# bensonlzl/spaced-kmer-sketching

Measured on AMD Instinct MI355X. Metric: k-mers hashed/s + genome-pairs ANI/s at 1/2/4/8 MI355X; % HBM roofline, higher is better.
Workload: dtype u64; 1 GPU; config3: 1x3 Gb multi-contig genome per GPU, spaced seed w=31/k=21 (mask seed 0), FracMinHash 1/1000; builds_in_flight=3, genome_bytes=3000000024, windows_per_genome=2999036400, sketch_size=2998764, parallelism=genome-sharded x1

## Files before the change

### spaced-kmer-sketching_amd/csrc/scan.hip

```cpp
#include <hip/hip_runtime.h>

#include <cstdlib>

#include <cstdint>
#include <type_traits>

#include "sks_hash.hpp"
#include "sks_internal.hpp"

namespace sks {

namespace {

constexpr int kBlock = 256;
constexpr int kWPT = 16;
constexpr int kTile = kBlock * kWPT;
constexpr int kHaloWords = 4;
constexpr int kWords = kBlock + kHaloWords;
constexpr int kLoadVecs = (kWords * 16 + 16) / 16;
constexpr int kQCap = 2048;
#ifndef SKS_SCAN_QCAP
#define SKS_SCAN_QCAP 512
#endif
template <int MODE>
constexpr int qcap() { return MODE == kModeList ? kQCap : SKS_SCAN_QCAP; }
constexpr unsigned char kSep = '\n';

struct Geom {
  uint64_t win0;
  uint64_t seg_end;
  uint32_t seg;
};

__device__ __forceinline__ Geom tile_geom(const ScanParams& p, uint64_t tile, uint32_t& seg) {
  while (seg + 1 < p.n_seg && tile >= p.tile_prefix[seg + 1]) ++seg;
  Geom g;
  g.seg = seg;
  g.win0 = p.seg_begin[seg] + (tile - p.tile_prefix[seg]) * (uint64_t)kTile;
  g.seg_end = p.seg_end[seg];
  return g;
}

__device__ __forceinline__ uint4 load_vec(const uint8_t* __restrict__ seq, int64_t base, int k,
                                          int64_t seg_end) {
  int64_t a = base + 16 * (int64_t)k;
  if (a + 16 <= seg_end) return *reinterpret_cast<const uint4*>(seq + a);
  uint32_t wv[4];
#pragma unroll
  for (int q = 0; q < 4; ++q) {
    uint32_t v = 0;
#pragma unroll
    for (int b = 0; b < 4; ++b) {
      int64_t pos = a + 4 * q + b;
      uint32_t ch = pos < seg_end ? seq[pos] : kSep;
      v |= ch << (8 * b);
    }
    wv[q] = v;
  }
  return make_uint4(wv[0], wv[1], wv[2], wv[3]);
}

__device__ __forceinline__ uint32_t align_shift(const uint8_t* seq, uint64_t win0) {
  return (uint32_t)(((uintptr_t)seq + win0) & 15u);
}

__device__ __forceinline__ void encode4(uint32_t x, uint32_t& le8, uint32_t& inv4) {
  uint32_t low = x | 0x20202020u;
  uint32_t code = ((low >> 1) ^ (low >> 2)) & 0x03030303u;
  uint32_t expect = __builtin_amdgcn_perm(0u, 0x74676361u, code);
  uint32_t eq = expect ^ low;
  uint32_t t = (eq & 0x7F7F7F7Fu) + 0x7F7F7F7Fu;
  t = ~(t | eq | 0x7F7F7F7Fu);
  uint32_t bad = (~t) & 0x80808080u;
  inv4 = (bad * 0x00204081u) >> 28;
  uint32_t y = code | (code >> 6);
  le8 = (y | (y >> 12)) & 0xFFu;
}

__device__ __forceinline__ uint32_t funnel(uint32_t hi, uint32_t lo, uint32_t s) {
  return __builtin_amdgcn_alignbit(hi, lo, s);
}

template <bool ALIGNED>
__device__ __forceinline__ void pack16(const uint32_t (&x)[5], uint32_t sb, uint32_t& le,
                                       uint32_t& inv) {
  uint32_t w[4], g[4], sad = 0;
#pragma unroll
  for (int k = 0; k < 4; ++k) {
    w[k] = ALIGNED ? x[k] : funnel(x[k + 1], x[k], sb);
    const uint32_t low = w[k] | 0x20202020u;
    const uint32_t code = ((low >> 1) ^ (low >> 2)) & 0x03030303u;
    const uint32_t expect = __builtin_amdgcn_perm(0u, 0x74676361u, code);
    sad = __builtin_amdgcn_sad_u8(low, expect, sad);
    g[k] = code * 0x01041040u;
  }
  const uint32_t g01 = __builtin_amdgcn_perm(g[1], g[0], 0x0c0c0703u);
  const uint32_t g23 = __builtin_amdgcn_perm(g[3], g[2], 0x0c0c0703u);
  le = __builtin_amdgcn_perm(g23, g01, 0x05040100u);
  inv = 0;
  if (sad) {
#pragma unroll
    for (int k = 0; k < 4; ++k) {
      uint32_t le8, inv4;
      encode4(w[k], le8, inv4);
      inv |= inv4 << (4 * k);
    }
  }
}

__device__ __forceinline__ uint32_t rev_pairs(uint32_t x) {
  uint32_t r = __builtin_bitreverse32(x);
  return ((r >> 1) & 0x55555555u) | ((r & 0x55555555u) << 1);
}


template <int MODE>
struct Queue {
  uint64_t key[qcap<MODE>()];
  uint64_t val[MODE == kModeBottom ? qcap<MODE>() : 1];
  uint32_t n;
  unsigned long long base;
  unsigned long long wins;
};

template <int MODE>
__device__ __forceinline__ void emit(const ScanParams& p, Queue<MODE>& q, uint32_t seg,
                                     uint64_t key, uint64_t val) {
  uint32_t slot = atomicAdd(&q.n, 1u);
  if (slot < (uint32_t)qcap<MODE>()) {
    q.key[slot] = key;
    if constexpr (MODE == kModeBottom) q.val[slot] = val;
  } else {
    unsigned long long g = atomicAdd(&p.seg_count[seg], 1ull);
    if (g < p.seg_out_cap[seg]) {
      uint64_t o = p.seg_out_off[seg] + g;
      p.out_key[o] = key;
      if constexpr (MODE == kModeBottom) p.out_val[o] = val;
    }
  }
}

template <int MODE>
__device__ __forceinline__ void flush(const ScanParams& p, Queue<MODE>& q, uint32_t seg) {
  __syncthreads();
  if (threadIdx.x == 0 && q.wins) atomicAdd(&p.seg_windows[seg], q.wins);
  constexpr uint32_t cap = qcap<MODE>();
  uint32_t n = q.n < cap ? q.n : cap;
  if (n) {
    if (threadIdx.x == 0) q.base = atomicAdd(&p.seg_count[seg], (unsigned long long)n);
    __syncthreads();
    uint64_t base = q.base;
    uint64_t cap = p.seg_out_cap[seg];
    uint64_t off = p.seg_out_off[seg];
    for (uint32_t i = threadIdx.x; i < n; i += kBlock) {
      if (base + i < cap) {
        p.out_key[off + base + i] = q.key[i];
        if constexpr (MODE == kModeBottom) p.out_val[off + base + i] = q.val[i];
      }
    }
  }
  __syncthreads();
  if (threadIdx.x == 0) {
    q.n = 0;
    q.wins = 0;
  }
  __syncthreads();
}

__device__ __forceinline__ void add_windows(unsigned long long& wins, uint32_t cnt) {
  uint32_t v = cnt;
#pragma unroll
  for (int o = 32; o > 0; o >>= 1) v += __shfl_xor(v, o, 64);
  if ((threadIdx.x & 63) == 0 && v) atomicAdd(&wins, (unsigned long long)v);
}

template <int FLAVOUR>
__device__ __forceinline__ uint64_t fmh_narrow(const ScanParams& p, uint64_t c) {
  uint64_t h;
  if constexpr (FLAVOUR == 0) {
    h = hash_mix(c + kGolden32);
    h = hash_mix(h + kGolden32);
    h = hash_mix(h + (128 + kGolden32));
  } else {
    h = hash_bitset128<1>(c, 0);
  }
  return h ^ p.kconst;
}

__device__ __forceinline__ uint64_t mix3_head(uint64_t c) {
  uint64_t h = hash_mix(c + kGolden32);
  h = hash_mix(h + kGolden32);
  uint64_t x = h + (128 + kGolden32);
  x ^= x >> 32;
  x = mul_const<kMixMul>(x);
  return x ^ (x >> 32);
}

template <int MODE>
__device__ __forceinline__ bool keep_fmh(const ScanParams& p, uint64_t f, uint64_t thresh) {
  if constexpr (MODE != kModeBottom) return div_test(f, p.low_mask, p.high_mask, p.dinv, p.dlim);
  else return f <= thresh;
}

constexpr int kBeOff = 2;

#ifndef SKS_SCAN_MIN_WAVES
#define SKS_SCAN_MIN_WAVES 1
#endif

constexpr uint32_t kCandCap = 128;

template <int MODE, int FLAVOUR, int PRE = 0>
__global__ __launch_bounds__(kBlock, SKS_SCAN_MIN_WAVES) void scan_kernel(ScanParams p) {
  __shared__ uint32_t s_raw[kLoadVecs * 4];
  __shared__ uint32_t s_be[kWords + 2 + kBeOff];
  __shared__ uint32_t s_lc[kWords + 2];
  __shared__ uint32_t s_inv[kWords + 2];
  __shared__ Queue<MODE> q;
  __shared__ ulonglong2 s_cand[PRE ? (kBlock / 64) * kCandCap : 1];

  __shared__ unsigned long long s_next;

  const int tid = threadIdx.x;
  const bool dyn = p.tile_queue != nullptr;
  uint64_t t_begin, t_end;
  if (dyn) {
    t_begin = (uint64_t)blockIdx.x * p.chunk;
    t_end = min(t_begin + p.chunk, p.n_tiles);
  } else {
    t_begin = (uint64_t)blockIdx.x * p.n_tiles / gridDim.x;
    t_end = (uint64_t)(blockIdx.x + 1) * p.n_tiles / gridDim.x;
  }
  if (tid == 0) {
    q.n = 0;
    q.wins = 0;
  }
  if (t_begin >= t_end) return;
  unsigned long long grab = 0;

  const int w = p.w;
  const uint32_t dshift = 2 * (32 - w);
  const bool dword = dshift >= 32;
  const uint32_t dbits = dshift & 31;
  const uint64_t wmask_bits = (w >= 64) ? ~0ull : ((1ull << w) - 1);
  const uint64_t region_bits = (kWPT - 1 + w >= 64) ? ~0ull : ((1ull << (kWPT - 1 + w)) - 1);
  if (tid < kBeOff) s_be[tid] = 0;

  uint32_t seg_lo = 0, seg_hi = p.n_seg;
  while (seg_lo + 1 < seg_hi) {
    uint32_t mid = (seg_lo + seg_hi) >> 1;
    if (p.tile_prefix[mid] <= t_begin) seg_lo = mid; else seg_hi = mid;
  }
  uint32_t cur_seg = seg_lo, pf_seg = seg_lo;

  Geom pg = tile_geom(p, t_begin, pf_seg);
  int64_t pf_base = (int64_t)pg.win0 - align_shift(p.seq, pg.win0);
  uint4 v0 = load_vec(p.seq, pf_base, tid, (int64_t)pg.seg_end);
  uint4 v1 = make_uint4(0, 0, 0, 0);
  if (tid < kLoadVecs - kBlock) v1 = load_vec(p.seq, pf_base, kBlock + tid, (int64_t)pg.seg_end);

  uint32_t win_count = 0;
  uint32_t count_seg = cur_seg;

  for (uint64_t tile = t_begin; tile < t_end;) {
    Geom g = tile_geom(p, tile, cur_seg);
    if (g.seg != count_seg) {
      add_windows(q.wins, win_count);
      win_count = 0;
      flush<MODE>(p, q, count_seg);
      count_seg = g.seg;
    }
    const uint32_t shift = align_shift(p.seq, g.win0);
    const uint64_t thresh = (MODE == kModeBottom) ? p.seg_thresh[g.seg] : 0;
    const bool last_of_chunk = tile + 1 == t_end;
    if (dyn && tid == 0) {
      if (tile == t_begin)
        grab = (unsigned long long)gridDim.x * p.chunk + atomicAdd(p.tile_queue, (unsigned long long)p.chunk);
      if (last_of_chunk) s_next = grab;
    }

    reinterpret_cast<uint4*>(s_raw)[tid] = v0;
    if (tid < kLoadVecs - kBlock) reinterpret_cast<uint4*>(s_raw)[kBlock + tid] = v1;
    __syncthreads();
    const uint64_t next_tile = !last_of_chunk ? tile + 1 : dyn ? (uint64_t)s_next : p.n_tiles;

    {
      const uint32_t sb = (shift & 3) * 8;
      auto pack_words = [&](auto aligned) {
        for (int i = tid; i < kWords; i += kBlock) {
          const uint32_t wi = (16 * i + shift) >> 2;
          uint32_t x[5];
#pragma unroll
          for (int k = 0; k < 5; ++k) x[k] = (decltype(aligned)::value && k == 4) ? 0u : s_raw[wi + k];
          uint32_t le, inv;
          pack16<decltype(aligned)::value>(x, sb, le, inv);
          s_be[kBeOff + i] = rev_pairs(le);
          s_lc[i] = ~le;
          s_inv[i] = inv;
        }
      };
      if (sb == 0) pack_words(std::true_type{});
      else pack_words(std::false_type{});
    }
    __syncthreads();

    if (next_tile < (dyn ? p.n_tiles : t_end)) {
      Geom ng = tile_geom(p, next_tile, pf_seg);
      pf_base = (int64_t)ng.win0 - align_shift(p.seq, ng.win0);
      v0 = load_vec(p.seq, pf_base, tid, (int64_t)ng.seg_end);
      if (tid < kLoadVecs - kBlock) v1 = load_vec(p.seq, pf_base, kBlock + tid, (int64_t)ng.seg_end);
    }

    uint32_t be[5];
#pragma unroll
    for (int k = 0; k < 5; ++k) be[k] = s_be[kBeOff + tid - 2 + k];
    uint32_t bs[3];
#pragma unroll
    for (int k = 0; k < 3; ++k) {
      const uint32_t hi = dword ? be[k] : be[k + 1];
      const uint32_t lo = dword ? be[k + 1] : be[k + 2];
      bs[k] = funnel(hi, lo, dbits);
    }
    const uint32_t lc0 = s_lc[tid], lc1 = s_lc[tid + 1], lc2 = s_lc[tid + 2];
    const uint64_t inv64 = (uint64_t)s_inv[tid] | ((uint64_t)s_inv[tid + 1] << 16) |
                           ((uint64_t)s_inv[tid + 2] << 32) | ((uint64_t)s_inv[tid + 3] << 48);
    const bool lane_clean = (inv64 & region_bits) == 0;
    auto canon = [&](uint32_t j) -> uint64_t {
      const uint32_t fh = j ? funnel(bs[0], bs[1], 32 - 2 * j) : bs[0];
      const uint32_t fl = j ? funnel(bs[1], bs[2], 32 - 2 * j) : bs[1];
      const uint64_t F = (((uint64_t)fh) << 32) | fl;
      const uint32_t rl = j ? funnel(lc1, lc0, 2 * j) : lc0;
      const uint32_t rh = j ? funnel(lc2, lc1, 2 * j) : lc1;
      const uint64_t R = (((uint64_t)rh) << 32) | rl;
      const uint64_t fm = F & p.mask_lo, rm = R & p.mask_lo;
      return fm < rm ? fm : rm;
    };
    if constexpr (PRE) {
      const int lane = tid & 63;
      ulonglong2* cb = s_cand + __builtin_amdgcn_readfirstlane(tid >> 6) * kCandCap;
      const uint32_t pmask = p.low_mask & 0xFu;
      const uint32_t kbits = (uint32_t)p.kconst & pmask;
      const uint32_t rest_lo = p.low_mask & ~0xFu, rest_hi = p.high_mask;
      uint32_t cnt = 0;
      auto finish = [&](uint32_t n) {
        __builtin_amdgcn_wave_barrier();
        if ((uint32_t)lane < n) {
          const ulonglong2 e = cb[lane];
          uint64_t y = mul_const<kMixMul>(e.x);
          y ^= y >> 28;
          const uint64_t f = y ^ p.kconst;
          bool keep = mul_uniform(f, p.dinv) <= p.dlim;
          if (rest_lo | rest_hi)
            keep = keep && ((((uint32_t)f & rest_lo) | ((uint32_t)(f >> 32) & rest_hi)) == 0);
          if (keep) emit<MODE>(p, q, g.seg, e.y, 0);
        }
        __builtin_amdgcn_wave_barrier();
      };
      auto window_pre = [&](auto checked, int j) {
          const uint64_t c = canon(j);
          const uint64_t z = mix3_head(c);
          const uint32_t ylo = (uint32_t)z * (uint32_t)kMixMul;
          bool pass = ((ylo ^ (ylo >> 28)) & pmask) == kbits;
          if constexpr (decltype(checked)::value) {
            const bool valid = ((inv64 >> j) & wmask_bits) == 0;
            win_count += valid ? 1u : 0u;
            pass = pass && valid;
          }
          const uint64_t bal = __ballot(pass);
          const uint32_t below = __builtin_amdgcn_mbcnt_hi(
              (uint32_t)(bal >> 32), __builtin_amdgcn_mbcnt_lo((uint32_t)bal, 0u));
          if (pass) cb[cnt + below] = make_ulonglong2(z, c);
          cnt += (uint32_t)__popcll(bal);
          if (cnt >= 64) {
            finish(64);
            const uint32_t rest = cnt - 64;
            ulonglong2 t = make_ulonglong2(0, 0);
            if ((uint32_t)lane < rest) t = cb[64 + lane];
            __builtin_amdgcn_wave_barrier();
            if ((uint32_t)lane < rest) cb[lane] = t;
            cnt = rest;
          }
      };
      if (__all(lane_clean)) {
#pragma unroll
        for (int j = 0; j < kWPT; ++j) window_pre(std::false_type{}, j);
        win_count += kWPT;
      } else {
#pragma unroll 1
        for (int j = 0; j < kWPT; ++j) window_pre(std::true_type{}, j);
      }
      if (cnt) finish(cnt);
    } else {
    uint32_t keepmask = 0;
    const uint32_t thr_top = (uint32_t)(thresh >> 36);
    const uint32_t k_top = (uint32_t)(p.kconst >> 32);
    auto keep_window = [&](uint64_t c) -> bool {
      if constexpr (MODE == kModeBottom && FLAVOUR == 0) {
        const uint64_t y = mul_const<kMixMul>(mix3_head(c));
        return (((uint32_t)(y >> 32) ^ k_top) >> 4) <= thr_top;
      } else {
        return keep_fmh<MODE>(p, fmh_narrow<FLAVOUR>(p, c), thresh);
      }
    };
    if (__all(lane_clean)) {
#pragma unroll
      for (int j = 0; j < kWPT; ++j) keepmask |= (keep_window(canon(j)) ? 1u : 0u) << j;
      win_count += kWPT;
    } else {
#pragma unroll 1
      for (int j = 0; j < kWPT; ++j) {
        const bool valid = ((inv64 >> j) & wmask_bits) == 0;
        win_count += valid ? 1u : 0u;
        keepmask |= (keep_window(canon(j)) && valid ? 1u : 0u) << j;
      }
    }
    while (keepmask) {
      const uint32_t j = __builtin_ctz(keepmask);
      keepmask &= keepmask - 1;
      if constexpr (MODE == kModeList) {
        emit<MODE>(p, q, g.seg, g.win0 + (uint64_t)(kWPT * tid) + j, 0);
      } else {
        const uint64_t c = canon(j);
        if constexpr (MODE == kModeFrac) emit<MODE>(p, q, g.seg, c, 0);
        else emit<MODE>(p, q, g.seg, c, c);
      }
    }
    }

    __syncthreads();
    if (q.n >= (uint32_t)qcap<MODE>() / 2) {
      add_windows(q.wins, win_count);
      win_count = 0;
      flush<MODE>(p, q, g.seg);
    }
    if (!last_of_chunk) {
      ++tile;
    } else if (dyn) {
      t_begin = tile = next_tile;
      t_end = min(next_tile + p.chunk, p.n_tiles);
    } else {
      break;
    }
  }
  add_windows(q.wins, win_count);
  flush<MODE>(p, q, count_seg);
}

template <int MODE, int FLAVOUR>
__global__ __launch_bounds__(kBlock) void scan_kernel_wide(ScanParams p) {
  __shared__ uint32_t s_raw[kLoadVecs * 4];
  __shared__ uint32_t s_be[kWords + 2];
  __shared__ uint32_t s_lc[kWords + 2];
  __shared__ uint32_t s_inv[kWords + 2];
  __shared__ uint64_t q_a[kQCap / 2], q_b[kQCap / 2], q_c[kQCap / 2];
  __shared__ uint32_t q_n;
  __shared__ unsigned long long q_base, q_wins;

  const int tid = threadIdx.x;
  const uint64_t t_begin = (uint64_t)blockIdx.x * p.n_tiles / gridDim.x;
  const uint64_t t_end = (uint64_t)(blockIdx.x + 1) * p.n_tiles / gridDim.x;
  if (tid == 0) {
    q_n = 0;
    q_wins = 0;
  }
  if (t_begin >= t_end) return;
  constexpr uint32_t cap = kQCap / 2;

  const int w = p.w;
  const uint32_t fshift = 128 - 2 * w;
  const uint64_t wmask_bits = (w >= 64) ? ~0ull : ((1ull << w) - 1);

  uint32_t seg_lo = 0, seg_hi = p.n_seg;
  while (seg_lo + 1 < seg_hi) {
    uint32_t mid = (seg_lo + seg_hi) >> 1;
    if (p.tile_prefix[mid] <= t_begin) seg_lo = mid; else seg_hi = mid;
  }
  uint32_t cur_seg = seg_lo, pf_seg = seg_lo;
  Geom pg = tile_geom(p, t_begin, pf_seg);
  int64_t pf_base = (int64_t)pg.win0 - align_shift(p.seq, pg.win0);
  uint4 v0 = load_vec(p.seq, pf_base, tid, (int64_t)pg.seg_end);
  uint4 v1 = make_uint4(0, 0, 0, 0);
  if (tid < kLoadVecs - kBlock) v1 = load_vec(p.seq, pf_base, kBlock + tid, (int64_t)pg.seg_end);
  uint32_t win_count = 0;
  uint32_t count_seg = cur_seg;

  auto wflush = [&](uint32_t seg) {
    __syncthreads();
    if (tid == 0 && q_wins) atomicAdd(&p.seg_windows[seg], q_wins);
    uint32_t n = q_n < cap ? q_n : cap;
    if (n) {
      if (tid == 0) q_base = atomicAdd(&p.seg_count[seg], (unsigned long long)n);
      __syncthreads();
      uint64_t base = q_base, c = p.seg_out_cap[seg], off = p.seg_out_off[seg];
      for (uint32_t i = tid; i < n; i += kBlock)
        if (base + i < c) {
          p.out_key[off + base + i] = q_a[i];
          if (MODE != kModeList) p.out_val[off + base + i] = q_b[i];
          if (MODE == kModeBottom) p.out_hi[off + base + i] = q_c[i];
        }
    }
    __syncthreads();
    if (tid == 0) {
      q_n = 0;
      q_wins = 0;
    }
    __syncthreads();
  };

  for (uint64_t tile = t_begin; tile < t_end; ++tile) {
    Geom g = tile_geom(p, tile, cur_seg);
    if (g.seg != count_seg) {
      add_windows(q_wins, win_count);
      win_count = 0;
      wflush(count_seg);
      count_seg = g.seg;
    }
    const uint32_t shift = align_shift(p.seq, g.win0);
    const uint64_t thresh = (MODE == kModeBottom) ? p.seg_thresh[g.seg] : 0;
    reinterpret_cast<uint4*>(s_raw)[tid] = v0;
    if (tid < kLoadVecs - kBlock) reinterpret_cast<uint4*>(s_raw)[kBlock + tid] = v1;
    __syncthreads();
    for (int i = tid; i < kWords; i += kBlock) {
      const uint32_t b0 = 16 * i + shift;
      const uint32_t wi = b0 >> 2, sb = (b0 & 3) * 8;
      uint32_t x[5];
#pragma unroll
      for (int k = 0; k < 5; ++k) x[k] = s_raw[wi + k];
      uint32_t le, inv;
      pack16<false>(x, sb, le, inv);
      s_be[i] = rev_pairs(le);
      s_lc[i] = ~le;
      s_inv[i] = inv;
    }
    __syncthreads();
    if (tile + 1 < t_end) {
      Geom ng = tile_geom(p, tile + 1, pf_seg);
      pf_base = (int64_t)ng.win0 - align_shift(p.seq, ng.win0);
      v0 = load_vec(p.seq, pf_base, tid, (int64_t)ng.seg_end);
      if (tid < kLoadVecs - kBlock) v1 = load_vec(p.seq, pf_base, kBlock + tid, (int64_t)ng.seg_end);
    }
    uint32_t be[5], lc[5];
#pragma unroll
    for (int k = 0; k < 5; ++k) { be[k] = s_be[tid + k]; lc[k] = s_lc[tid + k]; }
    const uint64_t inv_lo = (uint64_t)s_inv[tid] | ((uint64_t)s_inv[tid + 1] << 16) |
                            ((uint64_t)s_inv[tid + 2] << 32) | ((uint64_t)s_inv[tid + 3] << 48);
    const uint64_t inv_hi = (uint64_t)s_inv[tid + 4];
#pragma unroll
    for (int j = 0; j < kWPT; ++j) {
      uint32_t f3 = j ? funnel(be[0], be[1], 32 - 2 * j) : be[0];
      uint32_t f2 = j ? funnel(be[1], be[2], 32 - 2 * j) : be[1];
      uint32_t f1 = j ? funnel(be[2], be[3], 32 - 2 * j) : be[2];
      uint32_t f0 = j ? funnel(be[3], be[4], 32 - 2 * j) : be[3];
      uint64_t Fh = ((uint64_t)f3 << 32) | f2, Fl = ((uint64_t)f1 << 32) | f0;
      if (fshift) { Fl = (Fl >> fshift) | (Fh << (64 - fshift)); Fh >>= fshift; }
      uint32_t r0 = j ? funnel(lc[1], lc[0], 2 * j) : lc[0];
      uint32_t r1 = j ? funnel(lc[2], lc[1], 2 * j) : lc[1];
      uint32_t r2 = j ? funnel(lc[3], lc[2], 2 * j) : lc[2];
      uint32_t r3 = j ? funnel(lc[4], lc[3], 2 * j) : lc[3];
      uint64_t Rl = ((uint64_t)r1 << 32) | r0, Rh = ((uint64_t)r3 << 32) | r2;
      uint64_t fml = Fl & p.mask_lo, fmh = Fh & p.mask_hi;
      uint64_t rml = Rl & p.mask_lo, rmh = Rh & p.mask_hi;
      bool f_lt = (fmh < rmh) || (fmh == rmh && fml < rml);
      uint64_t cl = f_lt ? fml : rml, ch = f_lt ? fmh : rmh;
      uint64_t iv = (inv_lo >> j) | (j ? (inv_hi << (64 - j)) : 0);
      bool valid = (iv & wmask_bits) == 0;
      win_count += valid ? 1u : 0u;
      uint64_t h;
      if constexpr (FLAVOUR == 0) {
        h = hash_mix(cl + kGolden32);
        h = hash_mix(h + kGolden32 + ch);
        h = hash_mix(h + (128 + kGolden32));
      } else {
        h = hash_bitset128<1>(cl, ch);
      }
      uint64_t f = h ^ p.kconst;
      bool keep = (MODE != kModeBottom) ? div_test(f, p.low_mask, p.high_mask, p.dinv, p.dlim)
                                        : (f <= thresh);
      if (valid && keep) {
        uint32_t slot = atomicAdd(&q_n, 1u);
        uint64_t a = (MODE == kModeList) ? g.win0 + (uint64_t)(kWPT * tid) + j
                                         : (MODE == kModeFrac) ? cl : f;
        uint64_t b = (MODE == kModeFrac) ? ch : cl;
        if (slot < cap) {
          q_a[slot] = a; q_b[slot] = b; q_c[slot] = ch;
        } else {
          unsigned long long gi = atomicAdd(&p.seg_count[g.seg], 1ull);
          if (gi < p.seg_out_cap[g.seg]) {
            uint64_t o = p.seg_out_off[g.seg] + gi;
            p.out_key[o] = a;
            if (MODE != kModeList) p.out_val[o] = b;
            if (MODE == kModeBottom) p.out_hi[o] = ch;
          }
        }
      }
    }
    __syncthreads();
    if (q_n >= cap / 2) {
      add_windows(q_wins, win_count);
      win_count = 0;
      wflush(g.seg);
    }
  }
  add_windows(q_wins, win_count);
  wflush(count_seg);
}

constexpr int kGridOversubscribe = 16;
constexpr int kDynOversubscribe = 2;

template <class K>
int occupancy_grid(K kernel, int device) {
  int per_cu = 0;
  (void)hipOccupancyMaxActiveBlocksPerMultiprocessor(&per_cu, kernel, kBlock, 0);
  int cus = 0;
  (void)hipDeviceGetAttribute(&cus, hipDeviceAttributeMultiprocessorCount, device);
  if (per_cu < 1) per_cu = 1;
  if (cus < 1) cus = 1;
  return per_cu * cus;
}

}

uint64_t scan_tiles_for(uint64_t seg_bytes) { return (seg_bytes + kTile - 1) / kTile; }

hipError_t launch_scan(const ScanParams& p, int mode, int flavour, bool wide, int device,
                       hipStream_t stream, int grid_override) {
  if (p.n_tiles == 0) return hipSuccess;
  auto pick = [&](auto kernel) -> hipError_t {
    ScanParams q = p;
    q.tile_queue = nullptr;
    int grid = grid_override > 0 ? grid_override : kGridOversubscribe * occupancy_grid(kernel, device);
    if ((uint64_t)grid > p.n_tiles) grid = (int)p.n_tiles;
    hipLaunchKernelGGL(kernel, dim3(grid), dim3(kBlock), 0, stream, q);
    return hipGetLastError();
  };
  auto pick_dyn = [&](auto kernel) -> hipError_t {
    ScanParams q = p;
    int grid = grid_override > 0 ? grid_override : kDynOversubscribe * occupancy_grid(kernel, device);
    const uint64_t per = p.n_tiles / ((uint64_t)grid * 16);
    static const uint64_t min_chunk = getenv("SKS_SCAN_MIN_CHUNK") ? std::max(1, atoi(getenv("SKS_SCAN_MIN_CHUNK"))) : 3;
    q.chunk = (uint32_t)std::min<uint64_t>(16, std::max<uint64_t>(min_chunk, per));
    const uint64_t need = (p.n_tiles + q.chunk - 1) / q.chunk;
    if ((uint64_t)grid > need) grid = (int)need;
    hipLaunchKernelGGL(kernel, dim3(grid), dim3(kBlock), 0, stream, q);
    return hipGetLastError();
  };
  if (!wide && p.tile_queue) {
    if (mode == kModeFrac) {
      static const bool no_pre = getenv("SKS_NO_PREFILTER") != nullptr;
      if (flavour == 0 && (p.low_mask & 0xFu) && !no_pre) return pick_dyn(scan_kernel<kModeFrac, 0, 1>);
      return flavour == 0 ? pick_dyn(scan_kernel<kModeFrac, 0>) : pick_dyn(scan_kernel<kModeFrac, 1>);
    }
    if (mode == kModeBottom)
      return flavour == 0 ? pick_dyn(scan_kernel<kModeBottom, 0>) : pick_dyn(scan_kernel<kModeBottom, 1>);
  }
  if (!wide) {
    if (mode == kModeFrac) {
      static const bool no_pre = getenv("SKS_NO_PREFILTER") != nullptr;
      if (flavour == 0 && (p.low_mask & 0xFu) && !no_pre) return pick(scan_kernel<kModeFrac, 0, 1>);
      return flavour == 0 ? pick(scan_kernel<kModeFrac, 0>) : pick(scan_kernel<kModeFrac, 1>);
    }
    if (mode == kModeList) return flavour == 0 ? pick(scan_kernel<kModeList, 0>) : pick(scan_kernel<kModeList, 1>);
    return flavour == 0 ? pick(scan_kernel<kModeBottom, 0>) : pick(scan_kernel<kModeBottom, 1>);
  }
  if (mode == kModeFrac) return flavour == 0 ? pick(scan_kernel_wide<kModeFrac, 0>) : pick(scan_kernel_wide<kModeFrac, 1>);
  if (mode == kModeList) return flavour == 0 ? pick(scan_kernel_wide<kModeList, 0>) : pick(scan_kernel_wide<kModeList, 1>);
  return flavour == 0 ? pick(scan_kernel_wide<kModeBottom, 0>) : pick(scan_kernel_wide<kModeBottom, 1>);
}

SKS_CODE_OBJECT_HOOK(scan)

}
```

Measured before the change: 668.0 billion k-mers/s.

## Remap scan windows to strided lanes, pack aligned tiles from registers, tune occupancy

Each thread now handles windows with stride 16 across a 16-lane group instead of a contiguous run of 16 windows, and forms k-mers with a rolling funnel over shared words, so the per-lane 5-word preload and branchy shift selection go away. For aligned tiles the packing is done straight from the prefetched registers, which skips the raw shared-memory staging and one barrier. Clean-wave detection now checks inv words per wave rather than per-lane region bits. Launch-bounds min-waves defaults are raised per mode to trade registers for occupancy, with a risk of spills and of different shared-memory bank patterns.

```diff
diff --git a/spaced-kmer-sketching_amd/csrc/scan.hip b/spaced-kmer-sketching_amd/csrc/scan.hip
--- a/spaced-kmer-sketching_amd/csrc/scan.hip
+++ b/spaced-kmer-sketching_amd/csrc/scan.hip
@@ -204,14 +204,19 @@
 
 constexpr int kBeOff = 2;
 
-#ifndef SKS_SCAN_MIN_WAVES
-#define SKS_SCAN_MIN_WAVES 1
+template <int MODE, int PRE>
+constexpr int min_waves() {
+#ifdef SKS_SCAN_MIN_WAVES
+  return SKS_SCAN_MIN_WAVES;
+#else
+  return PRE ? 7 : MODE == kModeList ? 4 : 5;
 #endif
+}
 
 constexpr uint32_t kCandCap = 128;
 
 template <int MODE, int FLAVOUR, int PRE = 0>
-__global__ __launch_bounds__(kBlock, SKS_SCAN_MIN_WAVES) void scan_kernel(ScanParams p) {
+__global__ __launch_bounds__(kBlock, (min_waves<MODE, PRE>())) void scan_kernel(ScanParams p) {
   __shared__ uint32_t s_raw[kLoadVecs * 4];
   __shared__ uint32_t s_be[kWords + 2 + kBeOff];
   __shared__ uint32_t s_lc[kWords + 2];
@@ -240,11 +245,16 @@
 
   const int w = p.w;
   const uint32_t dshift = 2 * (32 - w);
-  const bool dword = dshift >= 32;
-  const uint32_t dbits = dshift & 31;
   const uint64_t wmask_bits = (w >= 64) ? ~0ull : ((1ull << w) - 1);
-  const uint64_t region_bits = (kWPT - 1 + w >= 64) ? ~0ull : ((1ull << (kWPT - 1 + w)) - 1);
   if (tid < kBeOff) s_be[tid] = 0;
+  const uint32_t r = tid & 15;
+  const uint32_t wbase = (uint32_t)(tid >> 4) * kWPT;
+  const uint32_t of = 2 * r + 64 - dshift;
+  const uint32_t qf = (of - 1) >> 5;
+  const uint32_t sF = 32 * qf + 32 - of;
+  const uint32_t sR = 2 * r;
+  const uint32_t* const fb = s_be + (kBeOff - 2) + wbase + qf;
+  const uint32_t* const rb = s_lc + wbase;
 
   uint32_t seg_lo = 0, seg_hi = p.n_seg;
   while (seg_lo + 1 < seg_hi) {
@@ -279,30 +289,43 @@
       if (last_of_chunk) s_next = grab;
     }
 
-    reinterpret_cast<uint4*>(s_raw)[tid] = v0;
-    if (tid < kLoadVecs - kBlock) reinterpret_cast<uint4*>(s_raw)[kBlock + tid] = v1;
-    __syncthreads();
-    const uint64_t next_tile = !last_of_chunk ? tile + 1 : dyn ? (uint64_t)s_next : p.n_tiles;
-
-    {
+    auto store_word = [&](int i, uint32_t le, uint32_t inv) {
+      s_be[kBeOff + i] = rev_pairs(le);
+      s_lc[i] = ~le;
+      s_inv[i] = inv;
+    };
+    if (shift == 0) {
+      uint32_t le, inv;
+      const uint32_t x0[5] = {v0.x, v0.y, v0.z, v0.w, 0u};
+      pack16<true>(x0, 0, le, inv);
+      store_word(tid, le, inv);
+      if (tid < kHaloWords) {
+        const uint32_t x1[5] = {v1.x, v1.y, v1.z, v1.w, 0u};
+        pack16<true>(x1, 0, le, inv);
+        store_word(kBlock + tid, le, inv);
+      }
+    } else {
+      reinterpret_cast<uint4*>(s_raw)[tid] = v0;
+      if (tid < kLoadVecs - kBlock) reinterpret_cast<uint4*>(s_raw)[kBlock + tid] = v1;
+      __syncthreads();
       const uint32_t sb = (shift & 3) * 8;
-      auto pack_words = [&](auto aligned) {
-        for (int i = tid; i < kWords; i += kBlock) {
-          const uint32_t wi = (16 * i + shift) >> 2;
-          uint32_t x[5];
-#pragma unroll
-          for (int k = 0; k < 5; ++k) x[k] = (decltype(aligned)::value && k == 4) ? 0u : s_raw[wi + k];
-          uint32_t le, inv;
-          pack16<decltype(aligned)::value>(x, sb, le, inv);
-          s_be[kBeOff + i] = rev_pairs(le);
-          s_lc[i] = ~le;
-          s_inv[i] = inv;
-        }
-      };
-      if (sb == 0) pack_words(std::true_type{});
-      else pack_words(std::false_type{});
-    }
-    __syncthreads();
+      for (int i = tid; i < kWords; i += kBlock) {
+        const uint32_t wi = (16 * i + shift) >> 2;
+        uint32_t x[5];
+#pragma unroll
+        for (int k = 0; k < 5; ++k) x[k] = s_raw[wi + k];
+        uint32_t le, inv;
+        pack16<false>(x, sb, le, inv);
+        store_word(i, le, inv);
+      }
+    }
+    __syncthreads();
+    uint64_t next_tile = !last_of_chunk ? tile + 1 : p.n_tiles;
+    if (last_of_chunk && dyn) {
+      const unsigned long long sn = s_next;
+      next_tile = ((uint64_t)__builtin_amdgcn_readfirstlane((uint32_t)(sn >> 32)) << 32) |
+                  __builtin_amdgcn_readfirstlane((uint32_t)sn);
+    }
 
     if (next_tile < (dyn ? p.n_tiles : t_end)) {
       Geom ng = tile_geom(p, next_tile, pf_seg);
@@ -311,32 +334,71 @@
       if (tid < kLoadVecs - kBlock) v1 = load_vec(p.seq, pf_base, kBlock + tid, (int64_t)ng.seg_end);
     }
 
-    uint32_t be[5];
-#pragma unroll
-    for (int k = 0; k < 5; ++k) be[k] = s_be[kBeOff + tid - 2 + k];
-    uint32_t bs[3];
-#pragma unroll
-    for (int k = 0; k < 3; ++k) {
-      const uint32_t hi = dword ? be[k] : be[k + 1];
-      const uint32_t lo = dword ? be[k + 1] : be[k + 2];
-      bs[k] = funnel(hi, lo, dbits);
-    }
-    const uint32_t lc0 = s_lc[tid], lc1 = s_lc[tid + 1], lc2 = s_lc[tid + 2];
-    const uint64_t inv64 = (uint64_t)s_inv[tid] | ((uint64_t)s_inv[tid + 1] << 16) |
-                           ((uint64_t)s_inv[tid + 2] << 32) | ((uint64_t)s_inv[tid + 3] << 48);
-    const bool lane_clean = (inv64 & region_bits) == 0;
-    auto canon = [&](uint32_t j) -> uint64_t {
-      const uint32_t fh = j ? funnel(bs[0], bs[1], 32 - 2 * j) : bs[0];
-      const uint32_t fl = j ? funnel(bs[1], bs[2], 32 - 2 * j) : bs[1];
+    const int lane = tid & 63;
+    bool dirty = s_inv[tid] != 0;
+    if (lane < 2) dirty = dirty || s_inv[(tid | 63) + 1 + lane] != 0;
+    const bool wave_clean = !__any(dirty);
+    auto canon_of = [&](uint32_t fh, uint32_t fl, uint32_t rh, uint32_t rl) -> uint64_t {
       const uint64_t F = (((uint64_t)fh) << 32) | fl;
-      const uint32_t rl = j ? funnel(lc1, lc0, 2 * j) : lc0;
-      const uint32_t rh = j ? funnel(lc2, lc1, 2 * j) : lc1;
       const uint64_t R = (((uint64_t)rh) << 32) | rl;
       const uint64_t fm = F & p.mask_lo, rm = R & p.mask_lo;
       return fm < rm ? fm : rm;
     };
+    auto canon_at = [&](uint32_t m) -> uint64_t {
+      const uint32_t f0 = fb[m], f1 = fb[m + 1], f2 = fb[m + 2];
+      const uint32_t r0 = rb[m], r1 = rb[m + 1], r2 = rb[m + 2];
+      return canon_of(funnel(f0, f1, sF), funnel(f1, f2, sF), funnel(r2, r1, sR), funnel(r1, r0, sR));
+    };
+    auto for_windows_checked = [&](auto body) {
+      const uint32_t* const ib = s_inv + wbase;
+      uint32_t fw = fb[1], rw = rb[1];
+      uint32_t fp = funnel(fb[0], fw, sF), rp = funnel(rw, rb[0], sR);
+      uint32_t i0 = ib[0], i1 = ib[1];
+      uint32_t fnext = 0, rnext = 0, inext = 0;
+      if constexpr (!PRE) {
+        fnext = fb[2];
+        rnext = rb[2];
+        inext = ib[2];
+      }
+#pragma unroll 1
+      for (int m = 0; m < kWPT; ++m) {
+        uint32_t fw2, rw2, i2;
+        if constexpr (PRE) {
+          fw2 = fb[m + 2];
+          rw2 = rb[m + 2];
+          i2 = ib[m + 2];
+        } else {
+          fw2 = fnext;
+          rw2 = rnext;
+          i2 = inext;
+          fnext = fb[m + 3];
+          rnext = rb[m + 3];
+          inext = ib[m + 3];
+        }
+        const uint32_t fn = funnel(fw, fw2, sF), rn = funnel(rw2, rw, sR);
+        const uint64_t iv = (uint64_t)i0 | ((uint64_t)i1 << 16) | ((uint64_t)i2 << 32);
+        body(m, canon_of(fp, fn, rn, rp), ((iv >> r) & wmask_bits) == 0);
+        fw = fw2; rw = rw2; fp = fn; rp = rn; i0 = i1; i1 = i2;
+      }
+    };
+    auto for_windows = [&](auto body) {
+      uint32_t fw = fb[1], rw = rb[1];
+      uint32_t fp = funnel(fb[0], fw, sF), rp = funnel(rw, rb[0], sR);
+      uint32_t fnext = fb[2], rnext = rb[2];
+#pragma unroll
+      for (int m = 0; m < kWPT; ++m) {
+        const uint32_t fw2 = fnext, rw2 = rnext;
+        if (m + 1 < kWPT) {
+          fnext = fb[m + 3];
+          rnext = rb[m + 3];
+        }
+        asm volatile("" ::: "memory");
+        const uint32_t fn = funnel(fw, fw2, sF), rn = funnel(rw2, rw, sR);
+        body(m, canon_of(fp, fn, rn, rp));
+        fw = fw2; rw = rw2; fp = fn; rp = rn;
+      }
+    };
     if constexpr (PRE) {
-      const int lane = tid & 63;
       ulonglong2* cb = s_cand + __builtin_amdgcn_readfirstlane(tid >> 6) * kCandCap;
       const uint32_t pmask = p.low_mask & 0xFu;
       const uint32_t kbits = (uint32_t)p.kconst & pmask;
@@ -356,16 +418,10 @@
         }
         __builtin_amdgcn_wave_barrier();
       };
-      auto window_pre = [&](auto checked, int j) {
-          const uint64_t c = canon(j);
+      auto window_pre = [&](uint64_t c, bool valid) {
           const uint64_t z = mix3_head(c);
           const uint32_t ylo = (uint32_t)z * (uint32_t)kMixMul;
-          bool pass = ((ylo ^ (ylo >> 28)) & pmask) == kbits;
-          if constexpr (decltype(checked)::value) {
-            const bool valid = ((inv64 >> j) & wmask_bits) == 0;
-            win_count += valid ? 1u : 0u;
-            pass = pass && valid;
-          }
+          const bool pass = (((ylo ^ (ylo >> 28)) & pmask) == kbits) && valid;
           const uint64_t bal = __ballot(pass);
           const uint32_t below = __builtin_amdgcn_mbcnt_hi(
               (uint32_t)(bal >> 32), __builtin_amdgcn_mbcnt_lo((uint32_t)bal, 0u));
@@ -381,13 +437,14 @@
             cnt = rest;
           }
       };
-      if (__all(lane_clean)) {
-#pragma unroll
-        for (int j = 0; j < kWPT; ++j) window_pre(std::false_type{}, j);
+      if (wave_clean) {
+        for_windows([&](int, uint64_t c) { window_pre(c, true); });
         win_count += kWPT;
       } else {
-#pragma unroll 1
-        for (int j = 0; j < kWPT; ++j) window_pre(std::true_type{}, j);
+        for_windows_checked([&](int, uint64_t c, bool valid) {
+          win_count += valid ? 1u : 0u;
+          window_pre(c, valid);
+        });
       }
       if (cnt) finish(cnt);
     } else {
@@ -402,25 +459,22 @@
         return keep_fmh<MODE>(p, fmh_narrow<FLAVOUR>(p, c), thresh);
       }
     };
-    if (__all(lane_clean)) {
-#pragma unroll
-      for (int j = 0; j < kWPT; ++j) keepmask |= (keep_window(canon(j)) ? 1u : 0u) << j;
+    if (wave_clean) {
+      for_windows([&](int m, uint64_t c) { keepmask |= (keep_window(c) ? 1u : 0u) << m; });
       win_count += kWPT;
     } else {
-#pragma unroll 1
-      for (int j = 0; j < kWPT; ++j) {
-        const bool valid = ((inv64 >> j) & wmask_bits) == 0;
+      for_windows_checked([&](int m, uint64_t c, bool valid) {
         win_count += valid ? 1u : 0u;
-        keepmask |= (keep_window(canon(j)) && valid ? 1u : 0u) << j;
-      }
+        keepmask |= (keep_window(c) && valid ? 1u : 0u) << m;
+      });
     }
     while (keepmask) {
       const uint32_t j = __builtin_ctz(keepmask);
       keepmask &= keepmask - 1;
       if constexpr (MODE == kModeList) {
-        emit<MODE>(p, q, g.seg, g.win0 + (uint64_t)(kWPT * tid) + j, 0);
+        emit<MODE>(p, q, g.seg, g.win0 + (uint64_t)(16 * (wbase + j) + r), 0);
       } else {
-        const uint64_t c = canon(j);
+        const uint64_t c = canon_at(j);
         if constexpr (MODE == kModeFrac) emit<MODE>(p, q, g.seg, c, 0);
         else emit<MODE>(p, q, g.seg, c, c);
       }
```

Result: faster. 708.1 billion k-mers/s, median of 6 (+6.0%).
